# OrangeEarth15/3dgrut

Measured on AMD Instinct MI355X. Metric: train-step images/sec + render ms/frame, MipNeRF360 bicycle @1/2/4/8 GPU, higher is better.
Workload: dtype f32

## Files before the change

### 3dgrut_amd/_capi.py

```python
import ctypes as C
import os

HERE = os.path.dirname(os.path.abspath(__file__))
LIB_PATH = os.environ.get("GUT_HIP_LIB", os.path.join(HERE, "libgut_hip.so"))

GUT_ABI_VERSION = 6
GUT_NUM_KERNEL_TIMERS = 11
BWD_RAW_PARAMETER_GRADS = 1
BWD_COMPACT_RADIANCE_GRADS = 2
BWD_SKIP_EPILOGUE = 4
OPT_LAZY_TILE_ORDER = 1
ADAM_CLEAR_CONSUMED_GRADS = 1
GRADIENT_RECORD_FLOATS = 16
OPT_SORTED_REFERENCE_BACKWARD = 2
OPT_EARLY_EXTRA_PERCENT = 3
OPT_FORWARD_TILE_ORDER = 4
OPT_KERNEL_TIMING_SET = 5
OPT_DEBUG_REPLACE_SCRATCH = 100
KERNEL_TIMER_NAMES = ("project", "scan", "expand", "sort", "ranges", "render", "render_bwd", "project_bwd", "optimizer",
                      "optimizer_early", "optimizer_early_2")

SHUTTER_GLOBAL = 4
CAMERA_PINHOLE, CAMERA_FISHEYE = 0, 1

BUF = dict(tiles_count=0, tiles_offset=1, proj_pos=2, conic_opacity=3, extent=4, depth=5, feat=6,
           unsorted_keys=7, unsorted_ids=8, sorted_keys=9, sorted_ids=10, tile_ranges=11, grad_scratch=12,
           tile_traversed_fwd=13, tile_traversed_bwd=14, ordered_ids=15, packed_rows=16)


class GutCamera(C.Structure):
    _fields_ = [
        ("model", C.c_int32), ("shutter", C.c_int32),
        ("principal_point", C.c_float * 2), ("focal_length", C.c_float * 2),
        ("radial_coeffs", C.c_float * 6), ("tangential_coeffs", C.c_float * 2), ("thin_prism_coeffs", C.c_float * 4),
        ("max_angle", C.c_float), ("pose_start", C.c_float * 7), ("pose_end", C.c_float * 7),
        ("timestamp_start_us", C.c_int64), ("timestamp_end_us", C.c_int64),
    ]


class GutConfig(C.Structure):
    _fields_ = [
        ("abi_version", C.c_int32), ("enable_kernel_timings", C.c_int32), ("particle_radiance_sph_degree", C.c_int32),
        ("particle_kernel_degree", C.c_int32), ("k_buffer_size", C.c_int32), ("global_z_order", C.c_int32),
        ("n_rolling_shutter_iterations", C.c_int32), ("ut_require_all_sigma_points", C.c_int32),
        ("rect_bounding", C.c_int32), ("tight_opacity_bounding", C.c_int32), ("tile_based_culling", C.c_int32),
        ("enable_hitcounts", C.c_int32),
        ("particle_kernel_min_response", C.c_float), ("particle_kernel_min_alpha", C.c_float),
        ("particle_kernel_max_alpha", C.c_float), ("min_transmittance", C.c_float),
        ("ut_alpha", C.c_float), ("ut_beta", C.c_float), ("ut_kappa", C.c_float), ("ut_in_image_margin_factor", C.c_float),
    ]
# ... 137 lines not shown
```

### 3dgrut_amd/csrc/gut_api.cpp

```cpp
#include <hip/hip_runtime.h>

#include <cmath>
#include <cstdarg>
#include <cstdio>
#include <cstdlib>
#include <cstring>
#include <deque>
#include <mutex>
#include <new>
#include <string>

#include "gut_internal.h"

namespace {

thread_local std::string g_last_error;

int fail(const char* fmt, ...) {
    char buf[512];
    va_list ap;
    va_start(ap, fmt);
    vsnprintf(buf, sizeof(buf), fmt, ap);
    va_end(ap);
    g_last_error = buf;
// ... 94 lines not shown
    int device = 0;
    GutConfig cfg{};
    gut::RenderConsts consts{};
    std::mutex mu;

    DevBuf tiles_count, tiles_offset, proj_pos, conic_opacity, extent, depth, feat, grad16, scan_temp;
    float* stat_accum = nullptr;
    int32_t* stat_denom = nullptr;
    GutRegularisation reg{};
    float* pose_out = nullptr;
    DevBuf pose_partials;
    DevBuf cam_pos;
    DevBuf wave_sums, block_prefix, scan_total;
    bool timing_main_stream = true, timing_side_stream = true;
    bool dbg_offset_valid = false;
    DevBuf sph_widened, sph_grad_wide;
    DevBuf packed12;
    bool packed_valid = false;
    bool packed_raw = false;
    DevBuf keys_unsorted, keys_sorted, ids_unsorted, ids_sorted, sort_temp;
    DevBuf ids_ordered, dbg_keys_sorted, dbg_ids_sorted;
    DevBuf tile_entries, tile_start, tile_cursor;
    uint32_t tile_entries_zeroed = 0;
    bool dbg_unsorted_valid = false;
    bool lazy_enabled = true;
    bool sorted_reference_bwd = true;
    bool lazy_order = false;
    bool dbg_sorted_valid = false;
    DevBuf ranges, trav_fwd, trav_bwd, tile_order;
    DevBuf counters;
    uint32_t* host_count = nullptr;
    uint32_t* host_count_dev = nullptr;
    hipEvent_t count_event = nullptr;
    hipStream_t side_stream = nullptr;
    hipEvent_t ev_projected = nullptr, ev_early_done = nullptr;
    struct EarlyArgs {
        gut::OptimiserState state;
        gut::AdamSettings adam;
        gut::SideStreamBlocks blocks;
        GutLazyMoments lazy;
        GutRegularisation reg;
    } early_args{};
    bool marks_valid = false;
    DevBuf wave_walked;
    int early_extra_percent = 100;
    bool stats_early = false;
// ... 204 lines not shown
    if (e == hipSuccess) e = h->counters.ensure(sizeof(gut::Counters));
    if (e != hipSuccess) {
        delete h;
        return fail("gut_create: allocation failed: %s", hipGetErrorString(e));
    }
    if (cfg->enable_kernel_timings)
        for (auto& set : h->ring)
            for (auto& ev : set.e)
                if (hipEventCreateWithFlags(&ev, kTimingEvent) != hipSuccess) ev = nullptr;
    *out = h;
    return 0;
}

void gut_destroy(gut_handle h) {
    if (!h) return;
    DeviceGuard dev_guard;
    (void)dev_guard.set(h->device);
    (void)hipDeviceSynchronize();
    DevBuf* bufs[] = {&h->tiles_count, &h->tiles_offset, &h->proj_pos, &h->conic_opacity, &h->extent, &h->depth, &h->feat,
                      &h->grad16, &h->scan_temp, &h->keys_unsorted, &h->keys_sorted, &h->ids_unsorted, &h->ids_sorted,
                      &h->sort_temp, &h->ranges, &h->trav_fwd, &h->trav_bwd, &h->tile_order, &h->counters, &h->ids_ordered,
                      &h->dbg_keys_sorted, &h->dbg_ids_sorted, &h->zero_word, &h->tile_ordered, &h->wave_walked, &h->packed12, &h->walk_sums,
                      &h->wave_sums, &h->block_prefix, &h->scan_total, &h->sph_widened, &h->sph_grad_wide, &h->cam_pos,
                      &h->tile_entries, &h->tile_start, &h->tile_cursor, &h->pose_partials};
    for (DevBuf* b : bufs) b->release();
    if (h->host_count) (void)hipHostFree(h->host_count);
    if (h->count_event) (void)hipEventDestroy(h->count_event);
    if (h->ev_projected) (void)hipEventDestroy(h->ev_projected);
    if (h->ev_early_done) (void)hipEventDestroy(h->ev_early_done);
    if (h->ev_bwd_start) (void)hipEventDestroy(h->ev_bwd_start);
    if (h->side_stream) (void)hipStreamDestroy(h->side_stream);
    (void)drain_timers(h->fwd_timers);
    (void)drain_timers(h->bwd_timers);
    for (auto& set : h->ring)
        for (auto& ev : set.e)
            if (ev) (void)hipEventDestroy(ev);
    delete h;
}

static int trace_fwd_impl(gut_handle h, void* stream_, uint32_t frame_number, int32_t num_active_features, uint32_t num_particles,
                          const float* d_particle_density, const float* d_particle_radiance, int32_t width, int32_t height,
                          const float* d_ray_origin, const float* d_ray_direction, const GutCamera* camera,
                          float* d_ray_radiance_density, float* d_ray_hit_distance, float* d_ray_hit_count,
                          float* d_particle_visibility, const float* d_features_albedo);

static void update_fwd_order(gut_handle h) {
    if (!h->walk_sums.p) return;
// ... 91 lines not shown
        if (timing && h->kev[i]) (void)hipEventRecord(h->kev[i], s);
    };

    gut::FrameClears clears;
    clears.ranges = h->ranges.as<uint2>();
    clears.trav_bwd = h->trav_bwd.as<uint32_t>();
    clears.tiles = (uint32_t)tiles;
    if (n) {
        HIP_TRY(h->wave_walked.ensure(((size_t)n + gut::kBlock - 1) / gut::kBlock * (gut::kBlock / 64) + 64));
        clears.wave_walked = h->wave_walked.as<uint8_t>();
        HIP_TRY(h->cam_pos.ensure(64));
        clears.cam_pos = h->cam_pos.as<float>();
        if (h->lazy_enabled && h->cfg.k_buffer_size == 0) {
            const void* before = h->tile_entries.p;
            HIP_TRY(h->tile_entries.ensure(sizeof(uint32_t) * (size_t)tiles));
            HIP_TRY(h->tile_start.ensure(sizeof(uint32_t) * ((size_t)tiles + 1)));
            HIP_TRY(h->tile_cursor.ensure(sizeof(uint32_t) * (size_t)tiles));
            if (h->tile_entries.p != before) h->tile_entries_zeroed = 0;
            if (h->tile_entries_zeroed < (uint32_t)tiles) {
                HIP_TRY(hipMemsetAsync(h->tile_entries.p, 0, h->tile_entries.cap, s));
                h->tile_entries_zeroed = (uint32_t)(h->tile_entries.cap / sizeof(uint32_t));
            }
            clears.tile_entries = h->tile_entries.as<uint32_t>();
        }
    } else {
        HIP_TRY(hipMemsetAsync(h->trav_bwd.p, 0, sizeof(uint32_t) * (size_t)tiles, s));
        HIP_TRY(hipMemsetAsync(h->ranges.p, 0, sizeof(uint32_t) * 2 * (size_t)tiles, s));
    }
    mark(0);
    if (h->cfg.particle_radiance_sph_degree != 3 && n) {
        const uint32_t w = 3u * (uint32_t)((h->cfg.particle_radiance_sph_degree + 1) * (h->cfg.particle_radiance_sph_degree + 1));
        HIP_TRY(h->sph_widened.ensure(sizeof(float) * 48 * (size_t)n));
        gut::launch_resize_sph_rows(s, n, w, 48u, d_particle_radiance, h->sph_widened.as<float>());
        d_particle_radiance = h->sph_widened.as<float>();
    }
    gut::launch_project(s, v, h->consts, n, num_active_features, d_particle_density, d_particle_radiance,
                        h->tiles_count.as<uint32_t>(), h->proj_pos.as<float>(), h->conic_opacity.as<float>(),
                        h->extent.as<float>(), h->depth.as<float>(), h->feat.as<float>(), d_particle_visibility,
                        h->wave_sums.as<uint32_t>(), d_features_albedo, clears);
    mark(1);
    static const bool early_after_project = getenv("GUT_EARLY_AFTER_PROJECT") != nullptr;
    if (early_after_project) {
        if (!h->ev_projected) HIP_TRY(hipEventCreateWithFlags(&h->ev_projected, kOrderingEvent));
        HIP_TRY(hipEventRecord(h->ev_projected, s));
    }
    const int end_bit = 32 + (int)bit_width_u32((uint32_t)tiles);
    h->dbg_sorted_valid = false;
    h->dbg_unsorted_valid = false;
    h->dbg_ordered_valid = false;
    const uint32_t* d_count = n ? h->scan_total.as<uint32_t>() : h->zero_word.as<uint32_t>();
    h->dbg_offset_valid = false;
    uint32_t m = 0;
    bool count_pending = false;
    if (n) {
        gut::launch_scan_wave_sums(s, n, h->wave_sums.as<uint32_t>(), h->block_prefix.as<uint32_t>(), h->scan_total.as<uint32_t>(),
                                   h->host_count_dev, h->walk_sums.as<uint32_t>(), clears.tile_entries, (uint32_t)tiles,
                                   h->tile_start.as<uint32_t>(), h->tile_cursor.as<uint32_t>());
        if (!h->count_event) HIP_TRY(hipEventCreateWithFlags(&h->count_event, kOrderingEvent));
        HIP_TRY(hipEventRecord(h->count_event, s));
        count_pending = true;
    }
    mark(2);
    auto bin_and_render = [&](uint32_t sort_n, bool lazy) -> int {
        h->lazy_order = lazy;
        if (sort_n && lazy) {
            HIP_TRY(h->keys_sorted.ensure(sizeof(uint64_t) * (size_t)sort_n));
            HIP_TRY(h->ids_ordered.ensure(sizeof(uint32_t) * (size_t)sort_n));
            gut::launch_expand_grouped(s, v, h->consts, n, h->proj_pos.as<float>(), h->conic_opacity.as<float>(), h->extent.as<float>(),
                                       h->depth.as<float>(), (uint32_t)tiles, h->tile_start.as<uint32_t>(), h->tile_cursor.as<uint32_t>(),
                                       h->ranges.as<uint32_t>(), h->keys_sorted.as<uint64_t>(), sort_n);
            mark(3);
            mark(4);
        } else if (sort_n) {
            HIP_TRY(h->keys_unsorted.ensure(sizeof(uint64_t) * (size_t)sort_n));
            HIP_TRY(h->keys_sorted.ensure(sizeof(uint64_t) * (size_t)sort_n));
            HIP_TRY(h->ids_unsorted.ensure(sizeof(uint32_t) * (size_t)sort_n));
            HIP_TRY(h->ids_sorted.ensure(sizeof(uint32_t) * (size_t)sort_n));
            gut::launch_expand(s, v, h->consts, n, h->tiles_count.as<uint32_t>(), h->wave_sums.as<uint32_t>(),
                               h->block_prefix.as<uint32_t>(), d_count, h->proj_pos.as<float>(),
                               h->conic_opacity.as<float>(), h->extent.as<float>(), h->depth.as<float>(),
                               h->keys_unsorted.as<uint64_t>(), h->ids_unsorted.as<uint32_t>(), sort_n);
            mark(3);
            HIP_TRY(h->sort_temp.ensure(gut::sort_temp_bytes(sort_n, end_bit)));
            HIP_TRY(gut::run_sort(s, h->sort_temp.p, h->sort_temp.cap, h->keys_unsorted.as<uint64_t>(), h->keys_sorted.as<uint64_t>(),
                                  h->ids_unsorted.as<uint32_t>(), h->ids_sorted.as<uint32_t>(), sort_n, end_bit));
            mark(4);
            gut::launch_tile_ranges(s, sort_n, h->keys_sorted.as<uint64_t>(), h->ranges.as<uint32_t>());
        } else {
            mark(3);
            mark(4);
        }
        mark(5);
        if (!early_after_project) {
// ... 598 lines not shown
        h->marks_valid = true;
    }
    HIP_TRY(hipEventRecord(h->ev_bwd_start, s));
    HIP_TRY(hipStreamWaitEvent(h->side_stream, h->ev_bwd_start, 0));
    if (h->cfg.enable_kernel_timings != 0 && h->timing_side_stream && h->kev[7]) (void)hipEventRecord(h->kev[7], h->side_stream);
    gut::launch_adam_rows_without_gradient(h->side_stream, h->n, h->tiles_count.as<uint32_t>(), ea.state, ea.adam, ea.blocks,
                                           gut_make_lazy(&ea.lazy, ea.adam.step), gut_make_reg(&ea.reg));
    HIP_TRY(hipGetLastError());
    const bool timing = h->cfg.enable_kernel_timings != 0 && h->timing_side_stream && h->kev[14] && h->kev[15];
    if (timing) {
        (void)hipEventRecord(h->kev[15], h->side_stream);
        h->ring[h->ring_cur].early2 = h->kev[7] != nullptr;
    }
    HIP_TRY(hipEventRecord(h->ev_early_done, h->side_stream));
    return 0;
}

int gut_set_option(gut_handle h, int32_t option, int32_t value) {
    if (!h) return fail("gut_set_option: null handle");
    std::lock_guard<std::mutex> lock(h->mu);
    switch (option) {
    case GUT_OPT_LAZY_TILE_ORDER: h->lazy_enabled = value != 0; return 0;
    case GUT_OPT_SORTED_REFERENCE_BACKWARD: h->sorted_reference_bwd = value != 0; return 0;
    case GUT_OPT_KERNEL_TIMING_SET:
        if (value < 0 || value > 2) return fail("gut_set_option: GUT_OPT_KERNEL_TIMING_SET takes 0, 1 or 2");
        h->timing_main_stream = value == 0;
        h->timing_side_stream = value != 2;
        return 0;
    case GUT_OPT_FORWARD_TILE_ORDER:
        if (value < -1 || value > 1) return fail("gut_set_option: GUT_OPT_FORWARD_TILE_ORDER takes -1, 0 or 1");
        h->fwd_order_mode = value;
        return 0;
    case GUT_OPT_EARLY_EXTRA_PERCENT:
        if (value < 0 || value > 100) return fail("gut_set_option: GUT_OPT_EARLY_EXTRA_PERCENT takes 0..100");
        h->early_extra_percent = value;
        return 0;
    case GUT_OPT_DEBUG_REPLACE_SCRATCH: {
        DevBuf* bufs[] = {&h->tiles_count, &h->tiles_offset, &h->proj_pos, &h->conic_opacity, &h->extent, &h->depth, &h->feat,
                          &h->grad16, &h->scan_temp, &h->keys_unsorted, &h->keys_sorted, &h->ids_unsorted, &h->ids_sorted,
                          &h->sort_temp, &h->ids_ordered, &h->ranges, &h->trav_fwd, &h->trav_bwd, &h->tile_order, &h->tile_ordered};
        const int count = (int)(sizeof(bufs) / sizeof(bufs[0]));
        if (value < 0 || value >= count) return fail("gut_set_option: GUT_OPT_DEBUG_REPLACE_SCRATCH takes 0..%d", count - 1);
        DevBuf& b = *bufs[value];
        if (!b.p) return 0;
        DeviceGuard dev_guard;
        HIP_TRY(dev_guard.set(h->device));
// ... 158 lines not shown
                hipError_t e = gut::run_sort(h->fwd_stream, tmp.p, tmp.cap, h->keys_unsorted.as<uint64_t>(),
                                             h->dbg_keys_sorted.as<uint64_t>(), h->ids_unsorted.as<uint32_t>(),
                                             h->dbg_ids_sorted.as<uint32_t>(), (uint32_t)m, h->end_bit);
                if (e == hipSuccess) e = hipStreamSynchronize(h->fwd_stream);
                tmp.release();
                HIP_TRY(e);
                h->dbg_sorted_valid = true;
            }
            if (which == GUT_BUF_SORTED_KEYS) { *d_ptr = h->dbg_keys_sorted.p; *bytes = 8 * m; }
            else { *d_ptr = h->dbg_ids_sorted.p; *bytes = 4 * m; }
        } else if (which == GUT_BUF_SORTED_KEYS) { *d_ptr = h->keys_sorted.p; *bytes = 8 * m; }
        else { *d_ptr = h->ids_sorted.p; *bytes = 4 * m; }
        break;
    case GUT_BUF_ORDERED_IDS:
        if (h->lazy_order && !h->dbg_ordered_valid && m) {
            DeviceGuard dev_guard;
            HIP_TRY(dev_guard.set(h->device));
            gut::launch_mask_unordered(h->fwd_stream, (uint32_t)h->tiles, h->ranges.as<uint32_t>(), h->tile_ordered.as<uint32_t>(),
                                       h->ids_ordered.as<uint32_t>());
            HIP_TRY(hipStreamSynchronize(h->fwd_stream));
            h->dbg_ordered_valid = true;
        }
        *d_ptr = h->lazy_order ? h->ids_ordered.p : h->ids_sorted.p; *bytes = 4 * m; break;
    case GUT_BUF_PACKED_ROWS:
        if (!h->packed_valid) return fail("gut_debug_buffer: the last forward was not a field-wise one (no packed rows)");
        *d_ptr = h->packed12.p; *bytes = 48 * n; break;
    case GUT_BUF_TILE_RANGES: *d_ptr = h->ranges.p; *bytes = 8 * t; break;
    case GUT_BUF_GRAD_SCRATCH:
        if (!h->have_backward) return fail("gut_debug_buffer: no backward yet");
        *d_ptr = h->grad16.p; *bytes = 64 * n; break;
    case GUT_BUF_TILE_TRAVERSED_FWD: *d_ptr = h->trav_fwd.p; *bytes = 4 * t; break;
    case GUT_BUF_TILE_TRAVERSED_BWD:
        if (!h->have_backward) return fail("gut_debug_buffer: no backward yet");
        *d_ptr = h->trav_bwd.p; *bytes = 4 * t; break;
    default: return fail("gut_debug_buffer: unknown buffer %d", which);
    }
    return 0;
}

int gut_debug_copy(gut_handle h, int32_t which, void* d_dst, size_t bytes) {
    void* src = nullptr;
    size_t have = 0;
    if (gut_debug_buffer(h, which, &src, &have)) return 1;
    if (bytes < have) return fail("gut_debug_copy: destination holds %zu bytes, buffer has %zu", bytes, have);
    if (have == 0) return 0;
    std::lock_guard<std::mutex> lock(h->mu);
// ... 9 lines not shown
```

### 3dgrut_amd/csrc/gut_internal.h

```cpp
#pragma once
#include <hip/hip_runtime.h>
#include <math.h>
#include <stdint.h>

#include "../../include/gut_hip.h"

namespace gut {

constexpr int kTile = 16;
constexpr int kBlock = 256;
constexpr uint32_t kInvalid = 0xFFFFFFFFu;

struct Affine {
    float r[3][3];
    float t[3];
};

struct ViewParams {
    Affine w2s_end;
    float pose_start[7], pose_end[7];
    int32_t shutter;
    Affine w2s_start;
    Affine w2s_mid;
    Affine s2w;
    int32_t model;
    int32_t width, height;
    int32_t grid_x, grid_y;
    float principal_point[2];
    float focal_length[2];
    float radial[6];
    float tangential[2];
    float thin_prism[4];
    float max_angle;
// ... 69 lines not shown
    const uint8_t* wave_walked = nullptr;
    uint32_t split_block = 0;
    uint32_t extra_end = 0;
    bool second_launch = false;
};
struct ScratchGradients {
    const float* camera_position = nullptr;
    float* grad16 = nullptr;
    const uint32_t* tiles_count = nullptr;
    const float* feat = nullptr;
};
struct PositionStatistics {
    float* accum = nullptr;
    int32_t* denom = nullptr;
};

struct FrameClears {
    uint2* ranges = nullptr;
    uint32_t* trav_bwd = nullptr;
    uint8_t* wave_walked = nullptr;
    uint32_t tiles = 0;
    float* cam_pos = nullptr;
    uint32_t* tile_entries = nullptr;
};

void launch_project(hipStream_t s, const ViewParams& v, const RenderConsts& c, uint32_t n, int sh_degree,
                    const float* density12, const float* sph48, uint32_t* tiles_count, float* proj_pos,
                    float* conic_opacity, float* extent, float* depth, float* feat, float* visibility,
                    uint32_t* wave_sums , const float* sph_albedo ,
                    const FrameClears& clears);
void launch_scan_wave_sums(hipStream_t s, uint32_t n, const uint32_t* wave_sums, uint32_t* block_prefix, uint32_t* total,
                           uint32_t* host_out , const uint32_t* walk_sums ,
                           uint32_t* tile_entries, uint32_t tiles, uint32_t* tile_start, uint32_t* tile_cursor);
void launch_expand_grouped(hipStream_t s, const ViewParams& v, const RenderConsts& c, uint32_t n, const float* proj_pos,
                           const float* conic_opacity, const float* extent, const float* depth, uint32_t tiles,
                           const uint32_t* tile_start, uint32_t* tile_cursor, uint32_t* ranges, uint64_t* entries, uint32_t capacity);
void launch_expand(hipStream_t s, const ViewParams& v, const RenderConsts& c, uint32_t n, const uint32_t* tiles_count,
                   const uint32_t* wave_sums, const uint32_t* block_prefix, const uint32_t* total , const float* proj_pos, const float* conic_opacity, const float* extent, const float* depth,
                   uint64_t* keys, uint32_t* ids, uint32_t capacity);
void launch_pad_keys(hipStream_t s, const uint32_t* count, uint32_t sort_n, uint64_t* keys, uint32_t* ids);
void launch_mask_unordered(hipStream_t s, uint32_t tiles, const uint32_t* ranges, const uint32_t* tile_ordered, uint32_t* ordered_ids);
void launch_tile_ranges(hipStream_t s, uint32_t m, const uint64_t* sorted_keys, uint32_t* ranges);
struct GradFields {
    float* pos = nullptr;
    float* dns = nullptr;
    float* rot = nullptr;
    float* scl = nullptr;
    float* alb = nullptr;
    float* spec = nullptr;
};
void launch_project_bwd(hipStream_t s, const ViewParams& v, uint32_t n, int sh_degree, const float* density12,
                        const uint32_t* tiles_count, const float* feat, float* grad16 ,
                        float* density_grad12, float* sph_grad48, bool raw_grads, const GradFields& fields = GradFields());
void launch_pack_fields(hipStream_t s, uint32_t n, const float* pos, const float* dns, const float* rot, const float* scl,
                        float* density12);
void launch_resize_sph_rows(hipStream_t s, uint32_t n, uint32_t in_width, uint32_t out_width, const float* in, float* out);
void launch_pack_activate_fields(hipStream_t s, uint32_t n, const float* pos, const float* dns_logit, const float* rot_raw,
                                 const float* log_scl, float* act12);

// ... 64 lines not shown
```

### 3dgrut_amd/csrc/gut_project.hip

```cpp
#include "gut_internal.h"

namespace gut {

__device__ __forceinline__ uint32_t f2u(float f) { return __float_as_uint(f); }
__device__ __forceinline__ float u2f(uint32_t u) { return __uint_as_float(u); }

__device__ float det_logf(float x) {
    uint32_t ix = f2u(x);
    int k = 0;
    if (ix >= 0x7f800000u) return x;
    if (ix < 0x00800000u) {
        if (ix == 0) return -__builtin_inff();
        x = x * 33554432.0f;
        ix = f2u(x);
        k -= 25;
    }
    k += (int)(ix >> 23) - 127;
    ix &= 0x007fffffu;
    const uint32_t i = (ix + (0x95f64u << 3)) & 0x800000u;
    x = u2f(ix | (i ^ 0x3f800000u));
    k += (int)(i >> 23);
    const float f = x - 1.0f;
    const float s = f / (2.0f + f);
    const float dk = (float)k;
// ... 251 lines not shown
    const float offx = tminx - mx, offy = tminy - my;
    const float lax = offx > 0.0f ? 1.0f : 0.0f, lay = offy > 0.0f ? 1.0f : 0.0f;
    const float nrx = lax + (mx > tmaxx ? 1.0f : 0.0f);
    const float nry = lay + (my > tmaxy ? 1.0f : 0.0f);
    if ((nrx + nry) > 0.0f) {
        const float px = lax > 0.0f ? tminx : tmaxx;
        const float py = lay > 0.0f ? tminy : tmaxy;
        const float dxx = copysignf(ts, offx), dxy = copysignf(ts, offy);
        const float dfx = mx - px, dfy = my - py;
        const float rcx = 1.0f / (ts * ts * c0);
        const float rcy = 1.0f / (ts * ts * c2);
        const float tx_ = nry * saturate((dxx * c0 * dfx + dxx * c1 * dfy) * rcx);
        const float ty_ = nrx * saturate((dxy * c1 * dfx + dxy * c2 * dfy) * rcy);
        const float qx = mx - (px + tx_ * dxx);
        const float qy = my - (py + ty_ * dxy);
        return 0.5f * (c0 * qx * qx + c2 * qy * qy) + c1 * qx * qy;
    }
    return 0.0f;
}

constexpr int kSerialTiles = 12;
constexpr int kShRow = 49;

constexpr int kBinWindow = 1536;

struct TileWindow {
    int x0, y0, w, h;
};

__device__ TileWindow tile_window(const TileBox& bb, bool small, uint32_t* bins, int* red , uint32_t tid) {
    constexpr int kNone = 0x7fffffff;
    int a = small ? bb.x0 : kNone, b = small ? bb.y0 : kNone, c = small ? -bb.x1 : kNone, d = small ? -bb.y1 : kNone;
#pragma unroll
    for (int o = 32; o > 0; o >>= 1) {
        a = min(a, __shfl_xor(a, o));
        b = min(b, __shfl_xor(b, o));
        c = min(c, __shfl_xor(c, o));
        d = min(d, __shfl_xor(d, o));
    }
    if ((tid & 63u) == 0u) {
        red[4 * (tid >> 6) + 0] = a;
        red[4 * (tid >> 6) + 1] = b;
        red[4 * (tid >> 6) + 2] = c;
        red[4 * (tid >> 6) + 3] = d;
    }
    __syncthreads();
    a = __builtin_amdgcn_readfirstlane(min(min(red[0], red[4]), min(red[8], red[12])));
// ... 168 lines not shown
        while (todo) {
            const int j = __ffsll((long long)todo) - 1;
            todo &= todo - 1;
            const int jx0 = bcast(bb.x0, j), jy0 = bcast(bb.y0, j), jw = bcast(bb.x1 - bb.x0, j), jarea = bcast(area, j);
            const float j0 = bcast(con0, j), j1 = bcast(con1, j), j2 = bcast(con2, j), jcx = bcast(cx, j), jcy = bcast(cy, j),
                        jmp = bcast(max_power, j);
            uint32_t total = 0;
            for (int base = 0; base < jarea; base += 64) {
                const int t = base + lane;
                bool pass = false;
                if (t < jarea) {
                    const int ty = t / jw;
                    const int tx = t - ty * jw;
                    pass = tile_min_power((float)(jx0 + tx), (float)(jy0 + ty), j0, j1, j2, jcx, jcy) < jmp;
                    if (pass) count_entry(jx0 + tx, jy0 + ty);
                }
                total += (uint32_t)__popcll(__ballot(pass));
            }
            if (lane == j) cnt = total;
        }
    }
    if (tile_entries) {
        __syncthreads();
        for (int k = (int)threadIdx.x; k < W.w * W.h; k += kBlock) {
            const uint32_t b = s_bins[k];
            if (b) atomicAdd(&tile_entries[window_tile(W, v.grid_x, (uint32_t)k)], b);
        }
    }

    const bool vis = cnt != 0;
    const unsigned long long vis_mask = __ballot(vis);
    if (vis_mask != 0ull) {
        float* wl = sh_lds + wave * 32 * kShRow;
        const float4* src = reinterpret_cast<const float4*>(sph48 + (size_t)wave_first * 48);
        float Y[16];
        float inv_dist = 0.f, dist = 0.f;
        if (vis) {
            const float rx = a.x - v.s2w.t[0], ry = a.y - v.s2w.t[1], rz = a.z - v.s2w.t[2];
            dist = sqrtf(rx * rx + ry * ry + rz * rz);
            inv_dist = 1.0f / dist;
            sh_basis(sh_degree, rx * inv_dist, ry * inv_dist, rz * inv_dist, Y);
        }
        const int ncoef = (sh_degree + 1) * (sh_degree + 1);
        float4 shq[12];
        float alb0 = 0.f, alb1 = 0.f, alb2 = 0.f;
        if (kSplitSH) {
            const float* spec = sph48 + (size_t)wave_first * 45;
            const uint32_t lim = rows_here * 45u;
            if (vis) {
// ... 269 lines not shown
            int tx = 0, ty = 0;
            if (t < jarea) {
                ty = t / jw;
                tx = t - ty * jw;
                pass = tile_min_power((float)(jx0 + tx), (float)(jy0 + ty), j0, j1, j2, jcx, jcy) < jmp;
            }
            const unsigned long long mask = __ballot(pass);
            const uint32_t my = joff + (uint32_t)__popcll(mask & ((1ull << lane) - 1ull));
            if (pass && my < jmax) {
                keys[my] = ((uint64_t)(uint32_t)((jy0 + ty) * v.grid_x + (jx0 + tx)) << 32) | jdkey;
                ids[my] = jid;
            }
            joff += (uint32_t)__popcll(mask);
        }
        if (lane == j) off = joff < jmax ? joff : jmax;
    }
    if (active)
        for (; off < max_off; ++off) {
            keys[off] = ((uint64_t)kInvalid << 32) | f2u(3.4028235e+38f);
            ids[off] = kInvalid;
        }
}

__global__ __launch_bounds__(kBlock) void k_expand_grouped(ViewParams v, RenderConsts c, uint32_t n,
                                                          const float2* __restrict__ proj_pos,
                                                          const float4* __restrict__ conic_opacity,
                                                          const float2* __restrict__ extent, const float* __restrict__ depth,
                                                          uint32_t tiles, const uint32_t* __restrict__ tile_start,
                                                          uint32_t* __restrict__ tile_cursor, uint2* __restrict__ ranges,
                                                          uint2* __restrict__ entries, uint32_t capacity) {
    __shared__ uint32_t s_bins[kBinWindow];
    __shared__ int s_red[16];
    const uint32_t i = blockIdx.x * kBlock + threadIdx.x;
    const int lane = (int)(threadIdx.x & 63);
    for (uint32_t t = i; t < tiles; t += gridDim.x * kBlock) {
        const uint32_t b = tile_start[t], e = tile_start[t + 1];
        ranges[t] = b == e ? make_uint2(0u, 0u) : make_uint2(min(b, capacity), min(e, capacity));
    }
    bool active = false;
    float2 e = make_float2(0.f, 0.f), p = make_float2(0.f, 0.f);
    float4 con = make_float4(0.f, 0.f, 0.f, 0.f);
    uint32_t dkey = 0;
    float max_power = 0.f;
    TileBox bb = {0, 0, 0, 0};
    int area = 0;
    if (i < n) {
        e = extent[i];
        active = !(e.x <= 1e-06f);
    }
    if (active) {
        dkey = f2u(depth[i]);
        p = proj_pos[i];
        bb = tile_bbox(v.grid_x, v.grid_y, p.x, p.y, e.x, e.y);
        area = (bb.x1 - bb.x0) * (bb.y1 - bb.y0);
        con = conic_opacity[i];
        if (c.tile_culling) max_power = det_logf(con.w / c.alpha_threshold);
    }
    const TileWindow W = tile_window(bb, active && area > 0 && area <= kSerialTiles, s_bins, s_red, threadIdx.x);
    auto enumerate = [&](auto emit) {
        if (!c.tile_culling) {
            if (active)
                for (int y = bb.y0; y < bb.y1; ++y)
                    for (int x = bb.x0; x < bb.x1; ++x) emit(x, y, i, dkey);
            return;
        }
        if (active && area <= kSerialTiles)
            for (int y = bb.y0; y < bb.y1; ++y)
                for (int x = bb.x0; x < bb.x1; ++x)
                    if (tile_min_power((float)x, (float)y, con.x, con.y, con.z, p.x, p.y) < max_power) emit(x, y, i, dkey);
        unsigned long long todo = __ballot(active && area > kSerialTiles);
        while (todo) {
            const int j = __ffsll((long long)todo) - 1;
            todo &= todo - 1;
            const int jx0 = bcast(bb.x0, j), jy0 = bcast(bb.y0, j), jw = bcast(bb.x1 - bb.x0, j), jarea = bcast(area, j);
            const float j0 = bcast(con.x, j), j1 = bcast(con.y, j), j2 = bcast(con.z, j), jcx = bcast(p.x, j), jcy = bcast(p.y, j),
                        jmp = bcast(max_power, j);
            const uint32_t jdkey = (uint32_t)bcast((int)dkey, j);
            const uint32_t jid = blockIdx.x * kBlock + (threadIdx.x & ~63u) + (uint32_t)j;
            for (int base = 0; base < jarea; base += 64) {
                const int t = base + lane;
                if (t < jarea) {
                    const int ty = t / jw;
                    const int tx = t - ty * jw;
                    if (tile_min_power((float)(jx0 + tx), (float)(jy0 + ty), j0, j1, j2, jcx, jcy) < jmp) emit(jx0 + tx, jy0 + ty, jid, jdkey);
                }
            }
        }
    };
    enumerate([&](int x, int y, uint32_t, uint32_t) {
        uint32_t bin;
        if (in_window(W, x, y, bin)) atomicAdd(&s_bins[bin], 1u);
    });
    __syncthreads();
    for (int k = (int)threadIdx.x; k < W.w * W.h; k += kBlock) {
        const uint32_t cnt = s_bins[k];
        if (cnt) s_bins[k] = atomicAdd(&tile_cursor[window_tile(W, v.grid_x, (uint32_t)k)], cnt);
    }
    __syncthreads();
    enumerate([&](int x, int y, uint32_t id, uint32_t dk) {
        uint32_t bin;
        const uint32_t slot = in_window(W, x, y, bin) ? atomicAdd(&s_bins[bin], 1u)
                                                      : atomicAdd(&tile_cursor[(uint32_t)y * (uint32_t)v.grid_x + (uint32_t)x], 1u);
        if (slot < capacity) entries[slot] = make_uint2(dk, id);
    });
}

__global__ __launch_bounds__(kBlock) void k_pad_keys(const uint32_t* __restrict__ count, uint32_t sort_n, uint64_t* __restrict__ keys,
                                                    uint32_t* __restrict__ ids) {
    const uint32_t m = *count;
    for (uint32_t k = m + blockIdx.x * kBlock + threadIdx.x; k < sort_n; k += gridDim.x * kBlock) {
        keys[k] = ((uint64_t)kInvalid << 32) | f2u(3.4028235e+38f);
        ids[k] = kInvalid;
    }
}

__global__ __launch_bounds__(kBlock) void k_mask_unordered(uint32_t tiles, const uint2* __restrict__ ranges,
                                                          const uint32_t* __restrict__ tile_ordered, uint32_t* __restrict__ ordered_ids) {
    const uint32_t t = blockIdx.x;
    if (t >= tiles) return;
// ... 229 lines not shown
    const int variant = v.model == GUT_CAMERA_OPENCV_FISHEYE ? 2 : (distorted ? 1 : 0);
    const bool rolling = v.shutter != GUT_SHUTTER_GLOBAL;
    auto kern = rolling ? (variant == 0 ? k_project_on_tiles<0, true, false> : (variant == 1 ? k_project_on_tiles<1, true, false> : k_project_on_tiles<2, true, false>))
                        : (variant == 0 ? k_project_on_tiles<0, false, false> : (variant == 1 ? k_project_on_tiles<1, false, false> : k_project_on_tiles<2, false, false>));
    if (sph_albedo)
        kern = rolling ? (variant == 0 ? k_project_on_tiles<0, true, true> : (variant == 1 ? k_project_on_tiles<1, true, true> : k_project_on_tiles<2, true, true>))
                       : (variant == 0 ? k_project_on_tiles<0, false, true> : (variant == 1 ? k_project_on_tiles<1, false, true> : k_project_on_tiles<2, false, true>));
    hipLaunchKernelGGL(kern, dim3(blocks_for(n)), dim3(kBlock), 0, s, v, c, n, sh_degree,
                       reinterpret_cast<const float4*>(density12), sph48, sph_albedo, tiles_count, reinterpret_cast<float2*>(proj_pos),
                       reinterpret_cast<float4*>(conic_opacity), reinterpret_cast<float2*>(extent), depth, feat, visibility,
                       wave_sums, clears);
}

void launch_scan_wave_sums(hipStream_t s, uint32_t n, const uint32_t* wave_sums, uint32_t* block_prefix, uint32_t* total,
                           uint32_t* host_out, const uint32_t* walk_sums, uint32_t* tile_entries, uint32_t tiles, uint32_t* tile_start,
                           uint32_t* tile_cursor) {
    if (n == 0) return;
    hipLaunchKernelGGL(k_scan_wave_sums, dim3(1), dim3(1024), 0, s, reinterpret_cast<const uint4*>(wave_sums), blocks_for(n), block_prefix,
                       total, host_out, walk_sums, tile_entries, tiles, tile_start, tile_cursor);
}

void launch_expand_grouped(hipStream_t s, const ViewParams& v, const RenderConsts& c, uint32_t n, const float* proj_pos,
                           const float* conic_opacity, const float* extent, const float* depth, uint32_t tiles,
                           const uint32_t* tile_start, uint32_t* tile_cursor, uint32_t* ranges, uint64_t* entries, uint32_t capacity) {
    if (n == 0) return;
    hipLaunchKernelGGL(k_expand_grouped, dim3(blocks_for(n)), dim3(kBlock), 0, s, v, c, n, reinterpret_cast<const float2*>(proj_pos),
                       reinterpret_cast<const float4*>(conic_opacity), reinterpret_cast<const float2*>(extent), depth, tiles, tile_start,
                       tile_cursor, reinterpret_cast<uint2*>(ranges), reinterpret_cast<uint2*>(entries), capacity);
}

void launch_expand(hipStream_t s, const ViewParams& v, const RenderConsts& c, uint32_t n, const uint32_t* tiles_count,
                   const uint32_t* wave_sums, const uint32_t* block_prefix, const uint32_t* total,
                   const float* proj_pos, const float* conic_opacity, const float* extent, const float* depth,
                   uint64_t* keys, uint32_t* ids, uint32_t capacity) {
    if (n == 0) return;
    hipLaunchKernelGGL(k_expand_tiles, dim3(blocks_for(n)), dim3(kBlock), 0, s, v, c, n, tiles_count,
                       reinterpret_cast<const uint4*>(wave_sums), block_prefix, total,
                       reinterpret_cast<const float2*>(proj_pos), reinterpret_cast<const float4*>(conic_opacity),
                       reinterpret_cast<const float2*>(extent), depth, keys, ids, capacity);
}

void launch_tile_ranges(hipStream_t s, uint32_t m, const uint64_t* sorted_keys, uint32_t* ranges) {
    if (m == 0) return;
    hipLaunchKernelGGL(k_tile_ranges, dim3(blocks_for(m)), dim3(kBlock), 0, s, m, sorted_keys,
                       reinterpret_cast<uint2*>(ranges));
}

void launch_project_bwd(hipStream_t s, const ViewParams& v, uint32_t n, int sh_degree, const float* density12,
                        const uint32_t* tiles_count, const float* feat, float* grad16, float* density_grad12,
                        float* sph_grad48, bool raw_grads, const GradFields& fields) {
    if (n == 0) return;
// ... 17 lines not shown
```

### 3dgrut_amd/tracer.py

```python
import ctypes as C
import enum
import math
import os

import numpy as np
import torch

from . import _capi
from .cameras import ShutterType as DatasetShutterType
from .pose import SensorPose3D, sensor_pose_from_c2w


class ShutterType(enum.IntEnum):
    ROLLING_TOP_TO_BOTTOM = 0
    ROLLING_LEFT_TO_RIGHT = 1
    ROLLING_BOTTOM_TO_TOP = 2
    ROLLING_RIGHT_TO_LEFT = 3
    GLOBAL = 4


SHUTTER_TYPE_MAP = {d: ShutterType[d.name] for d in DatasetShutterType}


def plugin_shutter_type(value):
# ... 414 lines not shown
        _capi.check(rc, "compact_gradient_rows")

    def collect_times(self):
        f, b = C.c_float(-1.0), C.c_float(-1.0)
        _capi.check(self._lib.gut_collect_times(self._handle, C.byref(f), C.byref(b)), "collect_times")
        if f.value >= 0:
            self._timings["forward_render"] = f.value
        if b.value >= 0:
            self._timings["backward_render"] = b.value
        return dict(self._timings)

    def set_lazy_tile_order(self, on=True):
        _capi.check(self._lib.gut_set_option(self._handle, _capi.OPT_LAZY_TILE_ORDER, 1 if on else 0), "set_option")

    def set_early_extra_percent(self, percent):
        _capi.check(self._lib.gut_set_option(self._handle, _capi.OPT_EARLY_EXTRA_PERCENT, int(percent)), "set_option")

    def set_forward_tile_order(self, mode):
        _capi.check(self._lib.gut_set_option(self._handle, _capi.OPT_FORWARD_TILE_ORDER, int(mode)), "set_option")

    def set_kernel_timing_set(self, which):
        _capi.check(self._lib.gut_set_option(self._handle, _capi.OPT_KERNEL_TIMING_SET, int(which)), "set_option")

    def debug_replace_scratch(self, index):
        _capi.check(self._lib.gut_set_option(self._handle, _capi.OPT_DEBUG_REPLACE_SCRATCH, int(index)), "set_option")

    def set_sorted_reference_backward(self, on=True):
        _capi.check(self._lib.gut_set_option(self._handle, _capi.OPT_SORTED_REFERENCE_BACKWARD, 1 if on else 0), "set_option")

    def stats(self):
        s = _capi.GutStats()
        _capi.check(self._lib.gut_get_stats(self._handle, C.byref(s)), "stats")
        return {k: int(getattr(s, k)) for k, _ in s._fields_ if k != "reserved"}

    def kernel_times(self):
        arr = (C.c_float * _capi.GUT_NUM_KERNEL_TIMERS)()
        _capi.check(self._lib.gut_kernel_times(self._handle, arr), "kernel_times")
        return dict(zip(_capi.KERNEL_TIMER_NAMES, [float(v) for v in arr]))

    def kernel_times_mean(self):
        arr = (C.c_float * _capi.GUT_NUM_KERNEL_TIMERS)()
        cnt = C.c_int32(0)
        _capi.check(self._lib.gut_kernel_times_mean(self._handle, arr, C.byref(cnt)), "kernel_times_mean")
        return dict(zip(_capi.KERNEL_TIMER_NAMES, [float(v) for v in arr])), int(cnt.value)

    def debug_buffer(self, name, device=None):
        ptr, nbytes = C.c_void_p(), C.c_size_t()
        _capi.check(self._lib.gut_debug_buffer(self._handle, _capi.BUF[name], C.byref(ptr), C.byref(nbytes)), "debug_buffer")
        dt = {"tiles_count": torch.int32, "tiles_offset": torch.int32, "unsorted_ids": torch.int32,
              "sorted_ids": torch.int32, "ordered_ids": torch.int32, "tile_ranges": torch.int32, "tile_traversed_fwd": torch.int32,
              "tile_traversed_bwd": torch.int32, "unsorted_keys": torch.int64,
              "sorted_keys": torch.int64}.get(name, torch.float32)
        n = nbytes.value // (8 if dt == torch.int64 else 4)
        dev = torch.device("cuda", self.device_index) if device is None else device
        out = torch.empty(n, dtype=dt, device=dev)
        if n:
            _capi.check(self._lib.gut_debug_copy(self._handle, _capi.BUF[name], C.c_void_p(out.data_ptr()),
                                                 C.c_size_t(nbytes.value)), "debug_copy")
        return out


class Tracer:
    class _Autograd(torch.autograd.Function):
        @staticmethod
        def forward(ctx, tracer_wrapper, frame_id, n_active_features, ray_ori, ray_dir, mog_pos, mog_rot, mog_scl,
                    mog_dns, mog_sph, sensor_params, sensor_poses, mog_sph_specular=None, raw_parameters=False):
            ctx.frame_id = frame_id
            ctx.n_active_features = n_active_features
            ctx.sensor_params = sensor_params
            ctx.sensor_poses = sensor_poses
            ctx.tracer_wrapper = tracer_wrapper
            ctx.set_materialize_grads(False)
            ctx.model_fields = mog_sph_specular is not None
            if ctx.model_fields:
# ... 144 lines not shown
```

### include/gut_hip.h

```cpp
#ifndef GUT_HIP_H
#define GUT_HIP_H

#include <stddef.h>
#include <stdint.h>

#ifdef __cplusplus
extern "C" {
#endif

#define GUT_ABI_VERSION 6

typedef struct gut_context* gut_handle;

enum { GUT_SHUTTER_ROLLING_TOP_TO_BOTTOM = 0, GUT_SHUTTER_ROLLING_LEFT_TO_RIGHT = 1,
       GUT_SHUTTER_ROLLING_BOTTOM_TO_TOP = 2, GUT_SHUTTER_ROLLING_RIGHT_TO_LEFT = 3, GUT_SHUTTER_GLOBAL = 4 };
enum { GUT_CAMERA_OPENCV_PINHOLE = 0, GUT_CAMERA_OPENCV_FISHEYE = 1 };

typedef struct GutCamera {
    int32_t model;
    int32_t shutter;
    float principal_point[2];
    float focal_length[2];
    float radial_coeffs[6];
    float tangential_coeffs[2];
// ... 35 lines not shown
    uint32_t sort_end_bit;
    uint32_t binning_overflows;
    uint64_t side_stream_rows;
    uint64_t side_stream_rows_first_launch;
} GutStats;

enum {
    GUT_BUF_TILES_COUNT = 0,
    GUT_BUF_TILES_OFFSET = 1,
    GUT_BUF_PROJ_POSITION = 2,
    GUT_BUF_CONIC_OPACITY = 3,
    GUT_BUF_PROJ_EXTENT = 4,
    GUT_BUF_GLOBAL_DEPTH = 5,
    GUT_BUF_FEATURES = 6,
    GUT_BUF_UNSORTED_KEYS = 7,
    GUT_BUF_UNSORTED_IDS = 8,
    GUT_BUF_SORTED_KEYS = 9,
    GUT_BUF_SORTED_IDS = 10,
    GUT_BUF_TILE_RANGES = 11,
    GUT_BUF_GRAD_SCRATCH = 12,
    GUT_BUF_TILE_TRAVERSED_FWD = 13,
    GUT_BUF_TILE_TRAVERSED_BWD = 14,
    GUT_BUF_ORDERED_IDS = 15,
    GUT_BUF_PACKED_ROWS = 16
};

void gut_default_config(GutConfig* cfg);

int gut_create(const GutConfig* cfg, int device_index, gut_handle* out);
void gut_destroy(gut_handle h);

int gut_trace(gut_handle h, void* stream, uint32_t frame_number, int32_t num_active_features ,
              uint32_t num_particles, const float* d_particle_density, const float* d_particle_radiance,
              int32_t width, int32_t height, const float* d_ray_origin, const float* d_ray_direction,
              const GutCamera* camera,
              float* d_ray_radiance_density, float* d_ray_hit_distance, float* d_ray_hit_count,
              float* d_particle_visibility);

int gut_trace_bwd(gut_handle h, void* stream, uint32_t frame_number, int32_t num_active_features,
                  uint32_t num_particles, const float* d_particle_density, const float* d_particle_radiance,
                  int32_t width, int32_t height, const float* d_ray_origin, const float* d_ray_direction,
                  const GutCamera* camera,
                  const float* d_ray_radiance_density, const float* d_ray_radiance_density_grad,
                  const float* d_ray_hit_distance, const float* d_ray_hit_distance_grad,
                  float* d_particle_density_grad, float* d_particle_radiance_grad);

#define GUT_BWD_RAW_PARAMETER_GRADS 1u
// ... 29 lines not shown
                               const float* d_positions, const float* d_density_logit, const float* d_rotation_raw, const float* d_log_scale,
                               const float* d_features_albedo, const float* d_features_specular, int32_t width, int32_t height,
                               const float* d_ray_origin, const float* d_ray_direction, const GutCamera* camera,
                               float* d_ray_radiance_density, float* d_ray_hit_distance, float* d_ray_hit_count,
                               float* d_particle_visibility);
int gut_trace_bwd_model_fields(gut_handle h, void* stream, uint32_t frame_number, int32_t num_active_features, uint32_t num_particles,
                               int32_t width, int32_t height, const float* d_ray_origin, const float* d_ray_direction,
                               const GutCamera* camera, const float* d_ray_radiance_density, const float* d_ray_radiance_density_grad,
                               const float* d_ray_hit_distance, const float* d_ray_hit_distance_grad, float* d_positions_grad,
                               float* d_density_grad, float* d_rotation_grad, float* d_scale_grad, float* d_features_albedo_grad,
                               float* d_features_specular_grad);

int gut_collect_times(gut_handle h, float* forward_render_ms, float* backward_render_ms);

int gut_get_stats(gut_handle h, GutStats* out);
int gut_debug_buffer(gut_handle h, int32_t which, void** d_ptr, size_t* bytes);
int gut_debug_copy(gut_handle h, int32_t which, void* d_dst, size_t bytes);

#define GUT_OPT_LAZY_TILE_ORDER 1
#define GUT_OPT_SORTED_REFERENCE_BACKWARD 2
#define GUT_OPT_EARLY_EXTRA_PERCENT 3
#define GUT_OPT_FORWARD_TILE_ORDER 4
#define GUT_OPT_KERNEL_TIMING_SET 5
#define GUT_OPT_DEBUG_REPLACE_SCRATCH 100
int gut_set_option(gut_handle h, int32_t option, int32_t value);

#define GUT_NUM_KERNEL_TIMERS 11
int gut_kernel_times(gut_handle h, float* ms8);
int gut_kernel_times_mean(gut_handle h, float* ms8, int32_t* count);

size_t gut_ssim_workspace_bytes(int32_t channels, int32_t height, int32_t width);
int gut_ssim_forward(void* stream, int32_t channels, int32_t height, int32_t width, int64_t stride_c, int64_t stride_h,
                     int64_t stride_w, const float* d_img1, const float* d_img2, void* d_workspace, float* d_mean_ssim);
int gut_ssim_backward(void* stream, int32_t channels, int32_t height, int32_t width, int64_t stride_c, int64_t stride_h,
                      int64_t stride_w, const float* d_img1, const float* d_img2, const void* d_workspace,
                      const float* d_upstream, float* d_grad_img1);

size_t gut_photometric_workspace_bytes(int32_t height, int32_t width);
int gut_photometric_loss(void* stream, int32_t height, int32_t width, const float* d_rgba, const float* d_gt_rgb, float background,
                         float lambda_l1, float lambda_ssim, void* d_workspace, float* d_loss3, float* d_rgba_grad);

int gut_photometric_loss_masked(void* stream, int32_t height, int32_t width, const float* d_rgba, const float* d_gt_rgb,
                                const float* d_mask, float background, float lambda_l1, float lambda_ssim, void* d_workspace,
                                float* d_loss3, float* d_rgba_grad);

int gut_photometric_loss_background(void* stream, int32_t height, int32_t width, const float* d_rgba, const float* d_gt_rgb,
// ... 124 lines not shown
```

Before: 451.7.

## Stage per-block tile bin counts from projection to skip recount in grouped expansion

The projection kernel now writes each block's tile window and per-window bin counts to global buffers. The grouped expansion kernel reads them back instead of re-enumerating every particle's tiles and re-binning with shared-memory atomics before reserving cursor slots. This removes one full tile-enumeration pass from expansion, at the cost of extra global writes in projection, a per-block count buffer, and reliance on the block-to-particle mapping matching between the two kernels.

Result: faster. 459.9, median of 6 (+1.8%).

```diff
diff --git a/3dgrut_amd/_capi.py b/3dgrut_amd/_capi.py
--- a/3dgrut_amd/_capi.py
+++ b/3dgrut_amd/_capi.py
@@ -16,6 +16,7 @@
 OPT_EARLY_EXTRA_PERCENT = 3
 OPT_FORWARD_TILE_ORDER = 4
 OPT_KERNEL_TIMING_SET = 5
+OPT_STAGED_EXPANSION = 6
 OPT_DEBUG_REPLACE_SCRATCH = 100
 KERNEL_TIMER_NAMES = ("project", "scan", "expand", "sort", "ranges", "render", "render_bwd", "project_bwd", "optimizer",
                       "optimizer_early", "optimizer_early_2")
@@ -25,7 +26,7 @@
 
 BUF = dict(tiles_count=0, tiles_offset=1, proj_pos=2, conic_opacity=3, extent=4, depth=5, feat=6,
            unsorted_keys=7, unsorted_ids=8, sorted_keys=9, sorted_ids=10, tile_ranges=11, grad_scratch=12,
-           tile_traversed_fwd=13, tile_traversed_bwd=14, ordered_ids=15, packed_rows=16)
+           tile_traversed_fwd=13, tile_traversed_bwd=14, ordered_ids=15, packed_rows=16, grouped_entries=17)
 
 
 class GutCamera(C.Structure):
diff --git a/3dgrut_amd/csrc/gut_api.cpp b/3dgrut_amd/csrc/gut_api.cpp
--- a/3dgrut_amd/csrc/gut_api.cpp
+++ b/3dgrut_amd/csrc/gut_api.cpp
@@ -140,6 +140,8 @@
     DevBuf ids_ordered, dbg_keys_sorted, dbg_ids_sorted;
     DevBuf tile_entries, tile_start, tile_cursor;
     uint32_t tile_entries_zeroed = 0;
+    DevBuf bin_window, bin_counts;
+    bool staged_expansion = true;
     bool dbg_unsorted_valid = false;
     bool lazy_enabled = true;
     bool sorted_reference_bwd = true;
@@ -390,7 +392,7 @@
                       &h->sort_temp, &h->ranges, &h->trav_fwd, &h->trav_bwd, &h->tile_order, &h->counters, &h->ids_ordered,
                       &h->dbg_keys_sorted, &h->dbg_ids_sorted, &h->zero_word, &h->tile_ordered, &h->wave_walked, &h->packed12, &h->walk_sums,
                       &h->wave_sums, &h->block_prefix, &h->scan_total, &h->sph_widened, &h->sph_grad_wide, &h->cam_pos,
-                      &h->tile_entries, &h->tile_start, &h->tile_cursor, &h->pose_partials};
+                      &h->tile_entries, &h->tile_start, &h->tile_cursor, &h->pose_partials, &h->bin_window, &h->bin_counts};
     for (DevBuf* b : bufs) b->release();
     if (h->host_count) (void)hipHostFree(h->host_count);
     if (h->count_event) (void)hipEventDestroy(h->count_event);
@@ -528,6 +530,13 @@
                 h->tile_entries_zeroed = (uint32_t)(h->tile_entries.cap / sizeof(uint32_t));
             }
             clears.tile_entries = h->tile_entries.as<uint32_t>();
+            if (h->staged_expansion) {
+                const size_t blocks = ((size_t)n + gut::kBlock - 1) / gut::kBlock;
+                HIP_TRY(h->bin_window.ensure(sizeof(int4) * blocks));
+                HIP_TRY(h->bin_counts.ensure(sizeof(uint16_t) * gut::kBinWindow * blocks));
+                clears.bin_window = h->bin_window.as<int4>();
+                clears.bin_counts = h->bin_counts.as<uint16_t>();
+            }
         }
     } else {
         HIP_TRY(hipMemsetAsync(h->trav_bwd.p, 0, sizeof(uint32_t) * (size_t)tiles, s));
@@ -574,7 +583,8 @@
             HIP_TRY(h->ids_ordered.ensure(sizeof(uint32_t) * (size_t)sort_n));
             gut::launch_expand_grouped(s, v, h->consts, n, h->proj_pos.as<float>(), h->conic_opacity.as<float>(), h->extent.as<float>(),
                                        h->depth.as<float>(), (uint32_t)tiles, h->tile_start.as<uint32_t>(), h->tile_cursor.as<uint32_t>(),
-                                       h->ranges.as<uint32_t>(), h->keys_sorted.as<uint64_t>(), sort_n);
+                                       h->ranges.as<uint32_t>(), h->keys_sorted.as<uint64_t>(), sort_n,
+                                       clears.bin_window, clears.bin_counts);
             mark(3);
             mark(4);
         } else if (sort_n) {
@@ -1219,6 +1229,9 @@
     switch (option) {
     case GUT_OPT_LAZY_TILE_ORDER: h->lazy_enabled = value != 0; return 0;
     case GUT_OPT_SORTED_REFERENCE_BACKWARD: h->sorted_reference_bwd = value != 0; return 0;
+    case GUT_OPT_STAGED_EXPANSION:
+        h->staged_expansion = value != 0;
+        return 0;
     case GUT_OPT_KERNEL_TIMING_SET:
         if (value < 0 || value > 2) return fail("gut_set_option: GUT_OPT_KERNEL_TIMING_SET takes 0, 1 or 2");
         h->timing_main_stream = value == 0;
@@ -1423,6 +1436,9 @@
             h->dbg_ordered_valid = true;
         }
         *d_ptr = h->lazy_order ? h->ids_ordered.p : h->ids_sorted.p; *bytes = 4 * m; break;
+    case GUT_BUF_GROUPED_ENTRIES:
+        if (!h->lazy_order) return fail("gut_debug_buffer: the last forward did not bin by tile (no grouped entries)");
+        *d_ptr = h->keys_sorted.p; *bytes = 8 * m; break;
     case GUT_BUF_PACKED_ROWS:
         if (!h->packed_valid) return fail("gut_debug_buffer: the last forward was not a field-wise one (no packed rows)");
         *d_ptr = h->packed12.p; *bytes = 48 * n; break;
diff --git a/3dgrut_amd/csrc/gut_internal.h b/3dgrut_amd/csrc/gut_internal.h
--- a/3dgrut_amd/csrc/gut_internal.h
+++ b/3dgrut_amd/csrc/gut_internal.h
@@ -9,6 +9,7 @@
 
 constexpr int kTile = 16;
 constexpr int kBlock = 256;
+constexpr int kBinWindow = 1536;
 constexpr uint32_t kInvalid = 0xFFFFFFFFu;
 
 struct Affine {
@@ -124,6 +125,8 @@
     uint32_t tiles = 0;
     float* cam_pos = nullptr;
     uint32_t* tile_entries = nullptr;
+    int4* bin_window = nullptr;
+    uint16_t* bin_counts = nullptr;
 };
 
 void launch_project(hipStream_t s, const ViewParams& v, const RenderConsts& c, uint32_t n, int sh_degree,
@@ -136,7 +139,9 @@
                            uint32_t* tile_entries, uint32_t tiles, uint32_t* tile_start, uint32_t* tile_cursor);
 void launch_expand_grouped(hipStream_t s, const ViewParams& v, const RenderConsts& c, uint32_t n, const float* proj_pos,
                            const float* conic_opacity, const float* extent, const float* depth, uint32_t tiles,
-                           const uint32_t* tile_start, uint32_t* tile_cursor, uint32_t* ranges, uint64_t* entries, uint32_t capacity);
+                           const uint32_t* tile_start, uint32_t* tile_cursor, uint32_t* ranges, uint64_t* entries, uint32_t capacity,
+                           const int4* bin_window ,
+                           const uint16_t* bin_counts);
 void launch_expand(hipStream_t s, const ViewParams& v, const RenderConsts& c, uint32_t n, const uint32_t* tiles_count,
                    const uint32_t* wave_sums, const uint32_t* block_prefix, const uint32_t* total , const float* proj_pos, const float* conic_opacity, const float* extent, const float* depth,
                    uint64_t* keys, uint32_t* ids, uint32_t capacity);
diff --git a/3dgrut_amd/csrc/gut_project.hip b/3dgrut_amd/csrc/gut_project.hip
--- a/3dgrut_amd/csrc/gut_project.hip
+++ b/3dgrut_amd/csrc/gut_project.hip
@@ -297,7 +297,6 @@
 constexpr int kSerialTiles = 12;
 constexpr int kShRow = 49;
 
-constexpr int kBinWindow = 1536;
 
 struct TileWindow {
     int x0, y0, w, h;
@@ -512,9 +511,12 @@
     }
     if (tile_entries) {
         __syncthreads();
+        uint16_t* const bin_counts = clr.bin_counts ? clr.bin_counts + (size_t)blockIdx.x * kBinWindow : nullptr;
+        if (bin_counts && threadIdx.x == 0) clr.bin_window[blockIdx.x] = make_int4(W.x0, W.y0, W.w, W.h);
         for (int k = (int)threadIdx.x; k < W.w * W.h; k += kBlock) {
             const uint32_t b = s_bins[k];
             if (b) atomicAdd(&tile_entries[window_tile(W, v.grid_x, (uint32_t)k)], b);
+            if (bin_counts) bin_counts[k] = (uint16_t)b;
         }
     }
 
@@ -830,17 +832,25 @@
         }
 }
 
+template <bool kTable>
 __global__ __launch_bounds__(kBlock) void k_expand_grouped(ViewParams v, RenderConsts c, uint32_t n,
                                                           const float2* __restrict__ proj_pos,
                                                           const float4* __restrict__ conic_opacity,
                                                           const float2* __restrict__ extent, const float* __restrict__ depth,
                                                           uint32_t tiles, const uint32_t* __restrict__ tile_start,
                                                           uint32_t* __restrict__ tile_cursor, uint2* __restrict__ ranges,
-                                                          uint2* __restrict__ entries, uint32_t capacity) {
+                                                          uint2* __restrict__ entries, uint32_t capacity,
+                                                          const int4* __restrict__ bin_window, const uint16_t* __restrict__ bin_counts) {
     __shared__ uint32_t s_bins[kBinWindow];
     __shared__ int s_red[16];
     const uint32_t i = blockIdx.x * kBlock + threadIdx.x;
     const int lane = (int)(threadIdx.x & 63);
+    int4 w4 = make_int4(0, 0, 0, 0);
+    uint32_t count0 = 0;
+    if (kTable) {
+        w4 = bin_window[blockIdx.x];
+        count0 = bin_counts[(size_t)blockIdx.x * kBinWindow + threadIdx.x];
+    }
     for (uint32_t t = i; t < tiles; t += gridDim.x * kBlock) {
         const uint32_t b = tile_start[t], e = tile_start[t + 1];
         ranges[t] = b == e ? make_uint2(0u, 0u) : make_uint2(min(b, capacity), min(e, capacity));
@@ -864,7 +874,6 @@
         con = conic_opacity[i];
         if (c.tile_culling) max_power = det_logf(con.w / c.alpha_threshold);
     }
-    const TileWindow W = tile_window(bb, active && area > 0 && area <= kSerialTiles, s_bins, s_red, threadIdx.x);
     auto enumerate = [&](auto emit) {
         if (!c.tile_culling) {
             if (active)
@@ -895,14 +904,28 @@
             }
         }
     };
-    enumerate([&](int x, int y, uint32_t, uint32_t) {
-        uint32_t bin;
-        if (in_window(W, x, y, bin)) atomicAdd(&s_bins[bin], 1u);
-    });
-    __syncthreads();
-    for (int k = (int)threadIdx.x; k < W.w * W.h; k += kBlock) {
-        const uint32_t cnt = s_bins[k];
-        if (cnt) s_bins[k] = atomicAdd(&tile_cursor[window_tile(W, v.grid_x, (uint32_t)k)], cnt);
+    TileWindow W = {0, 0, 0, 0};
+    if (kTable) {
+        const int wx = __builtin_amdgcn_readfirstlane(w4.x), wy = __builtin_amdgcn_readfirstlane(w4.y),
+                  ww = __builtin_amdgcn_readfirstlane(w4.z), wh = __builtin_amdgcn_readfirstlane(w4.w);
+        if (wx >= 0 && wy >= 0 && ww > 0 && wh > 0 && ww <= v.grid_x - wx && wh <= v.grid_y - wy && ww <= kBinWindow && wh <= kBinWindow &&
+            ww * wh <= kBinWindow)
+            W = TileWindow{wx, wy, ww, wh};
+        for (int k = (int)threadIdx.x; k < W.w * W.h; k += kBlock) {
+            const uint32_t cnt = k < kBlock ? count0 : bin_counts[(size_t)blockIdx.x * kBinWindow + k];
+            s_bins[k] = cnt ? atomicAdd(&tile_cursor[window_tile(W, v.grid_x, (uint32_t)k)], cnt) : 0u;
+        }
+    } else {
+        W = tile_window(bb, active && area > 0 && area <= kSerialTiles, s_bins, s_red, threadIdx.x);
+        enumerate([&](int x, int y, uint32_t, uint32_t) {
+            uint32_t bin;
+            if (in_window(W, x, y, bin)) atomicAdd(&s_bins[bin], 1u);
+        });
+        __syncthreads();
+        for (int k = (int)threadIdx.x; k < W.w * W.h; k += kBlock) {
+            const uint32_t cnt = s_bins[k];
+            if (cnt) s_bins[k] = atomicAdd(&tile_cursor[window_tile(W, v.grid_x, (uint32_t)k)], cnt);
+        }
     }
     __syncthreads();
     enumerate([&](int x, int y, uint32_t id, uint32_t dk) {
@@ -1178,11 +1201,13 @@
 
 void launch_expand_grouped(hipStream_t s, const ViewParams& v, const RenderConsts& c, uint32_t n, const float* proj_pos,
                            const float* conic_opacity, const float* extent, const float* depth, uint32_t tiles,
-                           const uint32_t* tile_start, uint32_t* tile_cursor, uint32_t* ranges, uint64_t* entries, uint32_t capacity) {
+                           const uint32_t* tile_start, uint32_t* tile_cursor, uint32_t* ranges, uint64_t* entries, uint32_t capacity,
+                           const int4* bin_window, const uint16_t* bin_counts) {
     if (n == 0) return;
-    hipLaunchKernelGGL(k_expand_grouped, dim3(blocks_for(n)), dim3(kBlock), 0, s, v, c, n, reinterpret_cast<const float2*>(proj_pos),
-                       reinterpret_cast<const float4*>(conic_opacity), reinterpret_cast<const float2*>(extent), depth, tiles, tile_start,
-                       tile_cursor, reinterpret_cast<uint2*>(ranges), reinterpret_cast<uint2*>(entries), capacity);
+    hipLaunchKernelGGL(bin_counts ? k_expand_grouped<true> : k_expand_grouped<false>, dim3(blocks_for(n)), dim3(kBlock), 0, s, v, c, n,
+                       reinterpret_cast<const float2*>(proj_pos), reinterpret_cast<const float4*>(conic_opacity),
+                       reinterpret_cast<const float2*>(extent), depth, tiles, tile_start, tile_cursor, reinterpret_cast<uint2*>(ranges),
+                       reinterpret_cast<uint2*>(entries), capacity, bin_window, bin_counts);
 }
 
 void launch_expand(hipStream_t s, const ViewParams& v, const RenderConsts& c, uint32_t n, const uint32_t* tiles_count,
diff --git a/3dgrut_amd/tracer.py b/3dgrut_amd/tracer.py
--- a/3dgrut_amd/tracer.py
+++ b/3dgrut_amd/tracer.py
@@ -460,6 +460,9 @@
     def set_kernel_timing_set(self, which):
         _capi.check(self._lib.gut_set_option(self._handle, _capi.OPT_KERNEL_TIMING_SET, int(which)), "set_option")
 
+    def set_staged_expansion(self, on=True):
+        _capi.check(self._lib.gut_set_option(self._handle, _capi.OPT_STAGED_EXPANSION, 1 if on else 0), "set_option")
+
     def debug_replace_scratch(self, index):
         _capi.check(self._lib.gut_set_option(self._handle, _capi.OPT_DEBUG_REPLACE_SCRATCH, int(index)), "set_option")
 
@@ -487,7 +490,7 @@
         _capi.check(self._lib.gut_debug_buffer(self._handle, _capi.BUF[name], C.byref(ptr), C.byref(nbytes)), "debug_buffer")
         dt = {"tiles_count": torch.int32, "tiles_offset": torch.int32, "unsorted_ids": torch.int32,
               "sorted_ids": torch.int32, "ordered_ids": torch.int32, "tile_ranges": torch.int32, "tile_traversed_fwd": torch.int32,
-              "tile_traversed_bwd": torch.int32, "unsorted_keys": torch.int64,
+              "tile_traversed_bwd": torch.int32, "unsorted_keys": torch.int64, "grouped_entries": torch.int64,
               "sorted_keys": torch.int64}.get(name, torch.float32)
         n = nbytes.value // (8 if dt == torch.int64 else 4)
         dev = torch.device("cuda", self.device_index) if device is None else device
diff --git a/include/gut_hip.h b/include/gut_hip.h
--- a/include/gut_hip.h
+++ b/include/gut_hip.h
@@ -81,7 +81,8 @@
     GUT_BUF_TILE_TRAVERSED_FWD = 13,
     GUT_BUF_TILE_TRAVERSED_BWD = 14,
     GUT_BUF_ORDERED_IDS = 15,
-    GUT_BUF_PACKED_ROWS = 16
+    GUT_BUF_PACKED_ROWS = 16,
+    GUT_BUF_GROUPED_ENTRIES = 17
 };
 
 void gut_default_config(GutConfig* cfg);
@@ -157,6 +158,7 @@
 #define GUT_OPT_EARLY_EXTRA_PERCENT 3
 #define GUT_OPT_FORWARD_TILE_ORDER 4
 #define GUT_OPT_KERNEL_TIMING_SET 5
+#define GUT_OPT_STAGED_EXPANSION 6
 #define GUT_OPT_DEBUG_REPLACE_SCRATCH 100
 int gut_set_option(gut_handle h, int32_t option, int32_t value);
 
```
